# orhosko/tiny-ntt

Measured on AMD Instinct MI355X. Metric: negacyclic poly-mults/sec (n=4096, 60-bit q), bit-exact vs cg_ntt.py, higher is better.
Workload: dtype u64; 1 GPU; n=4096, q=2^60-2^14+1 (60-bit), global batch 65536 = 65536 rows on this GPU, LCG-seeded rows resident in HBM (BASELINE configs[2]); n=4096, q=1152921504606830593, rows_per_gpu=65536, global_batch=65536, variant=fused, kernel=polymul_fused_kernel, lazy_reduction=True, lib_build_id=33db21926526ecac, parallelism=batch-sharded x1, no data-path collective

## Files before the change

### tiny_ntt_amd/csrc/fused_core.h

```cpp
#pragma once
#include <type_traits>
#include "modarith.h"

#ifndef TN_ABL_UNIFORM_TW
#define TN_ABL_UNIFORM_TW 0
#endif

namespace tn {

template <int B, int E_, typename F> struct StaticFor {
  TN_HD static void run(F& f) { f(std::integral_constant<int, B>()); StaticFor<B + 1, E_, F>::run(f); }
};
template <int E_, typename F> struct StaticFor<E_, E_, F> { TN_HD static void run(F&) {} };
template <int B, int E_, typename F> TN_HD void static_for(F&& f) { StaticFor<B, E_, F>::run(f); }

#ifndef TN_FUSED_LPT10
#define TN_FUSED_LPT10 3
#endif
#ifndef TN_FUSED_LPT12
#define TN_FUSED_LPT12 3
#endif
constexpr int fused_lpt(int logn) {
  return logn == 8 ? 2 : logn == 9 ? 3 : logn == 10 ? TN_FUSED_LPT10 : logn == 11 ? 3 : logn == 12 ? TN_FUSED_LPT12 : logn == 13 ? 3 : 0;
}

template <typename E> struct Arith {
  E q;
  u64 mu;
  int k;
  u32 fold_c;
  SplitK sk;
  u64 qmul[17];
  typename TwOf<E>::type one;
  typename TwOf<E>::type ninv;
  typename TwOf<E>::type fninv;
  typename TwOf<E>::type fninv_w1;
  typename TwOf<E>::type bninv;
  typename TwOf<E>::type bninv_w1;
};

template <typename E, int LOGN_, int LPT_> struct FusedCfg {
  static constexpr int LOGN = LOGN_, LPT = LPT_;
  static constexpr int N = 1 << LOGN, R = 1 << LPT, THREADS = N >> LPT;
  static constexpr int PHASES = (LOGN + LPT - 1) / LPT;
  static constexpr int pos(int p) { return (LOGN - (p + 1) * LPT) < 0 ? 0 : (LOGN - (p + 1) * LPT); }
  static constexpr int stage_begin(int p) { return p * LPT; }
  static constexpr int stage_end(int p) { return ((p + 1) * LPT) < LOGN ? ((p + 1) * LPT) : LOGN; }
  static constexpr int ex_pad(int e) { return pos(e + 1) > 0 ? (1 << pos(e + 1)) : 1; }
  static constexpr int ex_sh(int e) { return pos(e + 1) > 0 ? pos(e + 1) + LPT : LPT; }
  static constexpr int lay_span(int e, int cnt) { return cnt + ex_pad(e) * (cnt >> ex_sh(e)); }
  static constexpr int WB = (LOGN - LPT > 6) ? (LOGN - LPT - 6) : 0;
  static constexpr int WSH = LOGN - WB;
  static constexpr int tau_bit_to_j(int p, int t) { return t < pos(p) ? t : t + LPT; }
  static constexpr bool ex_wave_local(int e) {
    for (int t = 6; t < LOGN - LPT; ++t)
      if (tau_bit_to_j(e, t) != t + LPT || tau_bit_to_j(e + 1, t) != t + LPT) return false;
    return true;
  }
  static constexpr int region_elems() {
    int m = 1 << WSH;
    for (int e = 0; e + 1 < PHASES; ++e)
      if (ex_wave_local(e) && lay_span(e, 1 << WSH) > m) m = lay_span(e, 1 << WSH);
    return m;
  }
  static constexpr int lds_elems() {
    int m = region_elems() << WB;
    for (int e = 0; e + 1 < PHASES; ++e)
      if (!ex_wave_local(e) && lay_span(e, N) > m) m = lay_span(e, N);
    return m;
  }
  TN_HD static constexpr u32 jidx(int p, u32 tau, u32 r) {
    return ((tau >> pos(p)) << (pos(p) + LPT)) | (r << pos(p)) | (tau & ((1u << pos(p)) - 1u));
  }
  TN_HD static constexpr u32 ex_addr(int e, u32 j) {
    if (WB > 0 && ex_wave_local(e))
      return (j >> WSH) * (u32)region_elems() + (j & ((1u << WSH) - 1u)) + (u32)ex_pad(e) * ((j & ((1u << WSH) - 1u)) >> ex_sh(e));
    return j + (u32)ex_pad(e) * (j >> ex_sh(e));
  }
  TN_HD static constexpr u32 ex_base(int e, int p, u32 tau) { return ex_addr(e, jidx(p, tau, 0)); }
  TN_HD static constexpr u32 ex_off(int e, int p, u32 r) { return ex_addr(e, jidx(p, 0, r)); }
  enum { TW_UNIFORM = 0, TW_WAVE = 1, TW_LDS = 2, TW_REGS = 3, TW_VEC = 4 };
  static constexpr int LDS_TW_MAX_STAGE = 9;
  static constexpr int tw_src(int p) {
    return pos(p) >= LOGN - LPT ? TW_UNIFORM
         : (pos(p) >= 6 ? TW_WAVE : (pos(p) > 0 ? (stage_end(p) <= LDS_TW_MAX_STAGE ? TW_LDS : TW_VEC) : TW_REGS));
  }
  static constexpr int lds_tw_lo() {
    for (int p = 0; p < PHASES; ++p) if (tw_src(p) == TW_LDS) return 1 << stage_begin(p);
    return 0;
  }
  static constexpr int lds_tw_hi() {
    int h = 0;
    for (int p = 0; p < PHASES; ++p) if (tw_src(p) == TW_LDS) h = 1 << stage_end(p);
    return h;
  }
  static constexpr int lds_tw_count() { return lds_tw_hi() - lds_tw_lo(); }
  static constexpr int pre_count(int s) { return R >> ((LOGN - 1 - s) - pos(PHASES - 1) + 1); }
  static constexpr int pre_off(int s) {
    int o = 0;
    for (int i = stage_begin(PHASES - 1); i < s; ++i) o += pre_count(i);
    return o;
  }
  static constexpr int NPRE = (tw_src(PHASES - 1) == TW_REGS) ? pre_off(LOGN) : 1;
  TN_HD static u32 nat_addr(u32 k) { return k ^ ((k >> 5) & 15u); }
  TN_HD static u32 thi(int p, u32 tau) {
    if (pos(p) >= LOGN - LPT) return 0u;
    if (pos(p) >= 6) return wave_uniform(tau >> pos(p));
    return tau >> pos(p);
  }
};

template <typename E> struct LazyTraits;
template <> struct LazyTraits<u64> { static constexpr int LIMIT = 16, TMUL = 4, PW = 2; };
template <> struct LazyTraits<u32> { static constexpr int LIMIT = 64, TMUL = 2, PW = 4; };

template <typename E, bool LAZY, bool CIN = false> struct Policy {
  typedef typename TwOf<E>::type Tw;
  static constexpr bool lazy = LAZY;
  static constexpr bool canonical_inputs = CIN && LAZY && sizeof(E) == 8;
  static constexpr bool split = LAZY && sizeof(E) == 8;
  static constexpr int LIMIT = LazyTraits<E>::LIMIT, TMUL = LazyTraits<E>::TMUL, PW = LazyTraits<E>::PW;

  TN_HD static E load(E x, const Arith<E>& ar) {
    if (canonical_inputs) return x;
    if (LAZY) return fold(x, ar.k, ar.fold_c);
    return mul_tw(x, ar.one, ar.q);
  }
  TN_HD static E canon(E x, const Arith<E>& ar) {
    if (LAZY) { x = fold(x, ar.k, ar.fold_c); return csub(x, ar.q); }
    return x;
  }
  template <int K> TN_HD static void ct(E& u, E& v, Tw w, const Arith<E>& ar) {
    if constexpr (split) {
      const u64 x = mul_sp_acc(u, v, w, ar.sk);
      v = ((u << 1) + ar.qmul[K]) - x;
      u = x;
    } else if constexpr (LAZY) {
      const E t = mul_tw_lazy(v, w, ar.q);
      v = u + ((E)K * ar.q - t);
      u = u + t;
    } else {
      E t = mul_tw(v, w, ar.q);
      E s = u + t;
      v = u >= t ? u - t : u + (ar.q - t);
      u = csub(s, ar.q);
    }
  }
  template <int BND> TN_HD static void gs(E& u, E& v, Tw w, const Arith<E>& ar) {
    if constexpr (split) {
      const E d = (u + ar.qmul[BND]) - v;
      u = u + v;
      v = mul_sp(d, w, ar.sk);
    } else if constexpr (LAZY) {
      const E d = u + ((E)BND * ar.q - v);
      u = u + v;
      v = mul_tw_lazy(d, w, ar.q);
    } else {
      E d = u >= v ? u - v : u + (ar.q - v);
      u = csub(u + v, ar.q);
      v = mul_tw(d, w, ar.q);
    }
  }
  template <int BND> TN_HD static void gs_last(E& u, E& v, const Arith<E>& ar) {
    E d;
    if constexpr (split) d = (u + ar.qmul[BND]) - v;
    else d = LAZY ? (E)(u + ((E)BND * ar.q - v)) : (u >= v ? (E)(u - v) : (E)(u + (ar.q - v)));
    E s = u + v;
    u = mul_tw_canon(s, ar.fninv, ar);
    v = mul_tw_canon(d, ar.fninv_w1, ar);
  }
  TN_HD static E mul_tw_canon(E a, Tw w, const Arith<E>& ar) {
    if constexpr (split) return csub(fold(mul_sp(a, w, ar.sk), ar.k, ar.fold_c), ar.q);
    else return mul_tw(a, w, ar.q);
  }
};

template <typename P, int LOGN> struct Sched {
  static constexpr int fwd_in(int s) {
    int b = 2;
    for (int i = 0; i < s; ++i) { if (b + P::TMUL > P::LIMIT) b = 2; b += P::TMUL; }
    return b;
  }
  static constexpr bool fwd_fold(int s) { return P::lazy && fwd_in(s) + P::TMUL > P::LIMIT; }
  static constexpr int fwd_out() {
    int b = 2;
    for (int i = 0; i < LOGN; ++i) { if (b + P::TMUL > P::LIMIT) b = 2; b += P::TMUL; }
    return b;
  }
  static constexpr int inv_in(int g) {
    int b = P::lazy ? P::PW : 1;
    for (int i = 0; i < g; ++i) { if (2 * b > P::LIMIT) b = 2; b = (2 * b > P::TMUL) ? 2 * b : P::TMUL; }
    return b;
  }
  static constexpr bool inv_fold(int g) { return P::lazy && 2 * inv_in(g) > P::LIMIT; }
  static constexpr int inv_bnd(int g) { return inv_fold(g) ? 2 : inv_in(g); }
};

template <typename Cfg, bool CIN = false, bool BC = false> struct SplitSched {
  static constexpr int LOGN = Cfg::LOGN, R = Cfg::R;
  static constexpr int FEND = BC ? LOGN - 1 : LOGN;
  static constexpr long U = 4096, CAP = 16 * U;
  static constexpr long FOLDED = U + 1;
  static constexpr long PW_OUT = 2 * U;
  static constexpr long PW_IN = 14 * (U - 1);
  static constexpr long tmax(long bv) { return 4 * U + (bv + 7) / 8 + 2; }
  static constexpr long BC_AMAX = CAP - 8;
  static constexpr int kq(long b) { return (int)((b + U - 2) / (U - 1)); }
  static constexpr int kf(long t) { return kq(t) <= 6 ? 6 : kq(t); }
  static constexpr int ki(long b) { return (kq(b) + 3) / 4 * 4; }
  static constexpr int phase_of(int s) { return s / Cfg::LPT; }
  static constexpr int bpos_of(int s) { return (LOGN - 1 - s) - Cfg::pos(phase_of(s)); }
  struct Data {
    bool ffold[LOGN][R] = {};
    unsigned char fk[LOGN][R] = {};
    long fout = 0;
    bool pw_fold_b = false;
    bool bcfold[R] = {};
    bool ifold[LOGN][R] = {};
    unsigned char ik[LOGN][R] = {};
  };
  static constexpr Data build() {
    Data d;
    long b[R] = {};
    for (int r = 0; r < R; ++r) b[r] = CIN ? U : (r < R / 2 ? FOLDED : CAP);
    for (int s = 0; s < FEND; ++s) {
      if (s > 0 && phase_of(s) != phase_of(s - 1)) {
        long m = 0;
        for (int r = 0; r < R; ++r) m = b[r] > m ? b[r] : m;
        for (int r = 0; r < R; ++r) b[r] = m;
      }
      const int bit = 1 << bpos_of(s);
      for (int r = 0; r < R; ++r) {
        if (r & bit) continue;
        const long t = tmax(b[r | bit]);
        const int K = kf(t);
        const long grow = t > K * U ? t : K * U;
        if (b[r] + grow > CAP) { d.ffold[s][r] = true; b[r] = FOLDED; }
        d.fk[s][r] = (unsigned char)K;
        const long bu = b[r];
        b[r] = bu + t;
        b[r | bit] = bu + K * U;
      }
    }
    for (int r = 0; r < R; ++r) d.fout = b[r] > d.fout ? b[r] : d.fout;
    d.pw_fold_b = d.fout > PW_IN;
    for (int r = 0; r < R; r += 2) {
      if (!BC) { b[r] = b[r + 1] = PW_OUT; continue; }
      long a0 = b[r], a1 = b[r + 1];
      if (a0 > BC_AMAX) { d.bcfold[r] = true; a0 = FOLDED; }
      if (a1 > BC_AMAX) { d.bcfold[r + 1] = true; a1 = FOLDED; }
      b[r] = tmax(a0) + tmax(tmax(a1));
      b[r + 1] = tmax(a0) + tmax(a1);
    }
    for (int g = BC ? 1 : 0; g < LOGN; ++g) {
      const int s = LOGN - 1 - g;
      if (g > 0 && phase_of(s) != phase_of(s + 1)) {
        long m = 0;
        for (int r = 0; r < R; ++r) m = b[r] > m ? b[r] : m;
        for (int r = 0; r < R; ++r) b[r] = m;
      }
      const int bit = 1 << bpos_of(s);
      for (int r = 0; r < R; ++r) {
        if (r & bit) continue;
        const int v = r | bit;
        for (int it = 0; it < 2; ++it) {
          if (b[r] + ki(b[v]) * U <= CAP && b[r] + b[v] <= CAP) break;
          if (b[r] >= b[v]) { d.ifold[g][r] = true; b[r] = FOLDED; }
          else { d.ifold[g][v] = true; b[v] = FOLDED; }
        }
        const int Kv = ki(b[v]);
        d.ik[g][r] = (unsigned char)Kv;
        const long bd = b[r] + Kv * U;
        b[r] = b[r] + b[v];
        b[v] = tmax(bd);
      }
    }
    return d;
  }
  static constexpr Data D = build();
};

template <typename Pol, typename Cfg, bool BC = false> struct SchedOf {
  typedef Sched<Pol, Cfg::LOGN> S;
  static constexpr bool fwd_fold(int s, int r) { return S::fwd_fold(s) && !(r & (1 << SplitSched<Cfg>::bpos_of(s))); }
  static constexpr int fwd_k(int, int) { return Pol::TMUL; }
  static constexpr bool inv_fold(int g, int) { return S::inv_fold(g); }
  static constexpr int inv_k(int g, int) { return S::inv_bnd(g); }
  static constexpr bool pw_fold_b() { return false; }
  static constexpr bool pw_ok() { return !Pol::lazy || S::fwd_out() <= Pol::LIMIT - 2; }
};
template <typename Cfg, bool CIN, bool BC> struct SchedOf<Policy<u64, true, CIN>, Cfg, BC> {
  typedef SplitSched<Cfg, CIN, BC> S;
  static constexpr bool fwd_fold(int s, int r) { return S::D.ffold[s][r]; }
  static constexpr int fwd_k(int s, int r) { return S::D.fk[s][r]; }
  static constexpr bool inv_fold(int g, int r) { return S::D.ifold[g][r]; }
  static constexpr int inv_k(int g, int r) { return S::D.ik[g][r]; }
  static constexpr bool pw_fold_b() { return S::D.pw_fold_b; }
  static constexpr bool pw_ok() { return true; }
  static constexpr bool bc_fold(int r) { return S::D.bcfold[r]; }
};

template <typename E> struct TwRefs {
  typedef typename TwOf<E>::type Tw;
  const Tw* __restrict__ glob;
  const Tw* lds;
  Tw* pre;
  const Tw* mid = nullptr;
  u32 zero = 0;
};

template <typename E, typename Cfg, int PH, int S_>
TN_HD typename TwOf<E>::type tw_get(const TwRefs<E>& t, u32 thi, int g) {
  constexpr int bpos = (Cfg::LOGN - 1 - S_) - Cfg::pos(PH);
  if (Cfg::tw_src(PH) == Cfg::TW_REGS) return t.pre[Cfg::pre_off(S_) + g];
  const u32 idx = (1u << S_) + (TN_ABL_UNIFORM_TW ? 0u : (thi << (Cfg::LPT - bpos - 1))) + (u32)g;
  if (Cfg::tw_src(PH) == Cfg::TW_LDS) {
    if (t.mid) return t.mid[(1 << (S_ - Cfg::stage_begin(PH))) - 1 + g];
    return t.lds[idx - Cfg::lds_tw_lo()];
  }
  if (Cfg::tw_src(PH) == Cfg::TW_VEC && t.mid) return t.mid[(1 << (S_ - Cfg::stage_begin(PH))) - 1 + g];
  return t.glob[idx + t.zero];
}

template <typename E, typename Cfg, int PH>
TN_HD void tw_fetch_vec(typename TwOf<E>::type (&mid)[Cfg::R], u32 tau, const typename TwOf<E>::type* __restrict__ glob) {
  const u32 thi = Cfg::thi(PH, tau);
  static_for<Cfg::stage_begin(PH), Cfg::stage_end(PH)>([&](auto s_) {
    constexpr int s = decltype(s_)::value;
    constexpr int bpos = (Cfg::LOGN - 1 - s) - Cfg::pos(PH);
    constexpr int cnt = Cfg::R >> (bpos + 1), off = (1 << (s - Cfg::stage_begin(PH))) - 1;
    const u32 boff = ((1u << s) + (thi << (Cfg::LPT - bpos - 1))) * (u32)sizeof(typename TwOf<E>::type);
    const typename TwOf<E>::type* base = reinterpret_cast<const typename TwOf<E>::type*>(reinterpret_cast<const char*>(glob) + boff);
#pragma unroll
    for (int g = 0; g < cnt; ++g) mid[off + g] = base[g];
  });
}

template <typename E, typename Cfg, int PH>
TN_HD void tw_fetch_mid(typename TwOf<E>::type (&mid)[Cfg::R], u32 tau, const typename TwOf<E>::type* lds_tw) {
  const u32 thi = Cfg::thi(PH, tau);
  static_for<Cfg::stage_begin(PH), Cfg::stage_end(PH)>([&](auto s_) {
    constexpr int s = decltype(s_)::value;
    constexpr int bpos = (Cfg::LOGN - 1 - s) - Cfg::pos(PH);
    constexpr int cnt = Cfg::R >> (bpos + 1), off = (1 << (s - Cfg::stage_begin(PH))) - 1;
#pragma unroll
    for (int g = 0; g < cnt; ++g)
      mid[off + g] = lds_tw[(1u << s) + (thi << (Cfg::LPT - bpos - 1)) + (u32)g - Cfg::lds_tw_lo()];
  });
}

template <typename E, typename Cfg, int S0, int S1>
TN_HD void tw_prefetch_stages(typename TwOf<E>::type* pre, u32 tau, const typename TwOf<E>::type* __restrict__ glob) {
  constexpr int PH = Cfg::PHASES - 1;
  if (Cfg::tw_src(PH) != Cfg::TW_REGS) return;
  const u32 thi = Cfg::thi(PH, tau);
  static_for<S0, S1>([&](auto s_) {
    constexpr int s = decltype(s_)::value;
    constexpr int bpos = (Cfg::LOGN - 1 - s) - Cfg::pos(PH);
    const u32 off = ((1u << s) + (thi << (Cfg::LPT - bpos - 1))) * (u32)sizeof(typename TwOf<E>::type);
    const typename TwOf<E>::type* base = reinterpret_cast<const typename TwOf<E>::type*>(reinterpret_cast<const char*>(glob) + off);
#pragma unroll
    for (int g = 0; g < Cfg::pre_count(s); ++g) pre[Cfg::pre_off(s) + g] = base[g];
  });
}
template <typename E, typename Cfg>
TN_HD void tw_prefetch_raw(typename TwOf<E>::type* pre, u32 tau, const typename TwOf<E>::type* __restrict__ glob) {
  tw_prefetch_stages<E, Cfg, Cfg::stage_begin(Cfg::PHASES - 1), Cfg::LOGN>(pre, tau, glob);
}

template <typename E, typename Cfg>
TN_HD void tw_prefetch(typename TwOf<E>::type (&pre)[Cfg::NPRE], u32 tau, const typename TwOf<E>::type* __restrict__ glob) {
  tw_prefetch_raw<E, Cfg>(pre, tau, glob);
}

template <typename E, typename Cfg, typename Pol, int PH, bool BC = false>
TN_HD void fwd_phase(E (&x)[Cfg::R], u32 tau, const TwRefs<E>& tw, const Arith<E>& ar) {
  typedef SchedOf<Pol, Cfg, BC> SO;
  typedef typename TwOf<E>::type Tw;
  const u32 thi = Cfg::thi(PH, tau);
  constexpr int SEND = BC && Cfg::stage_end(PH) == Cfg::LOGN ? Cfg::LOGN - 1 : Cfg::stage_end(PH);
  static_for<Cfg::stage_begin(PH), SEND>([&](auto s_) {
    constexpr int s = decltype(s_)::value;
    constexpr int bpos = (Cfg::LOGN - 1 - s) - Cfg::pos(PH);
    static_for<0, Cfg::R>([&](auto r_) {
      constexpr int r = decltype(r_)::value;
      if constexpr (Pol::lazy && SO::fwd_fold(s, r)) x[r] = fold(x[r], ar.k, ar.fold_c);
    });
    static_for<0, Cfg::R>([&](auto r_) {
      constexpr int r = decltype(r_)::value;
      if constexpr (!(r & (1 << bpos))) {
        const Tw w = tw_get<E, Cfg, PH, s>(tw, thi, r >> (bpos + 1));
        Pol::template ct<SO::fwd_k(s, r)>(x[r], x[r | (1 << bpos)], w, ar);
      }
    });
  });
}

template <typename E, typename Cfg, typename Pol, int PH, bool BC = false>
TN_HD void inv_phase(E (&x)[Cfg::R], u32 tau, const TwRefs<E>& tw, const Arith<E>& ar) {
  typedef SchedOf<Pol, Cfg, BC> SO;
  typedef typename TwOf<E>::type Tw;
  const u32 thi = Cfg::thi(PH, tau);
  constexpr int SEND = BC && Cfg::stage_end(PH) == Cfg::LOGN ? Cfg::LOGN - 1 : Cfg::stage_end(PH);
  static_for<0, SEND - Cfg::stage_begin(PH)>([&](auto i_) {
    constexpr int s = SEND - 1 - decltype(i_)::value;
    constexpr int g = Cfg::LOGN - 1 - s;
    constexpr int bpos = (Cfg::LOGN - 1 - s) - Cfg::pos(PH);
    static_for<0, Cfg::R>([&](auto r_) {
      constexpr int r = decltype(r_)::value;
      if constexpr (Pol::lazy && SO::inv_fold(g, r)) x[r] = fold(x[r], ar.k, ar.fold_c);
    });
    static_for<0, Cfg::R>([&](auto r_) {
      constexpr int r = decltype(r_)::value;
      if constexpr (!(r & (1 << bpos))) {
        constexpr int BND = SO::inv_k(g, r);
        if constexpr (s == 0) Pol::template gs_last<BND>(x[r], x[r | (1 << bpos)], ar);
        else {
          const Tw w = tw_get<E, Cfg, PH, s>(tw, thi, r >> (bpos + 1));
          Pol::template gs<BND>(x[r], x[r | (1 << bpos)], w, ar);
        }
      }
    });
  });
}

template <typename E, typename Cfg, typename Pol>
TN_HD void load_reduce(E (&x)[Cfg::R], const Arith<E>& ar) {
#pragma unroll
  for (int r = 0; r < Cfg::R / 2; ++r) x[r] = Pol::load(x[r], ar);
}

template <typename E, typename Cfg, int EX, int PH>
TN_HD void ex_store(const E (&x)[Cfg::R], u32 tau, E* lds) {
  E* base = lds + Cfg::ex_base(EX, PH, tau);
  static_for<0, Cfg::R>([&](auto r_) { constexpr int r = decltype(r_)::value; base[Cfg::ex_off(EX, PH, r)] = x[r]; });
}
template <typename E, typename Cfg, int EX, int PH>
TN_HD void ex_load(E (&x)[Cfg::R], u32 tau, const E* lds) {
  const E* base = lds + Cfg::ex_base(EX, PH, tau);
  static_for<0, Cfg::R>([&](auto r_) { constexpr int r = decltype(r_)::value; x[r] = base[Cfg::ex_off(EX, PH, r)]; });
}

TN_HD u64 pointwise_lazy(u64 a, u64 b, const Arith<u64>& ar) {
  return mulmod_solinas_lazy(fold(a, ar.k, ar.fold_c), b, ar.k, ar.fold_c);
}
TN_HD u32 pointwise_lazy(u32 a, u32 b, const Arith<u32>& ar) {
  return mulmod_barrett_lazy(fold(a, ar.k, ar.fold_c), fold(b, ar.k, ar.fold_c), ar.q, ar.mu, ar.k);
}
template <typename E, typename Cfg, typename Pol>
TN_HD void pointwise(E (&xa)[Cfg::R], const E (&xb)[Cfg::R], const Arith<E>& ar) {
  typedef SchedOf<Pol, Cfg> SO;
  static_assert(SO::pw_ok(), "pointwise_lazy: unfolded operand bound");
#pragma unroll
  for (int r = 0; r < Cfg::R; ++r) {
    if (Pol::lazy)
      xa[r] = pointwise_lazy(xa[r], SO::pw_fold_b() ? fold(xb[r], ar.k, ar.fold_c) : xb[r], ar);
    else
      xa[r] = mulmod_barrett(xa[r], xb[r], ar.q, ar.mu, ar.k);
    if (r & 1) sched_fence();
  }
}

TN_HD void basecase_pair(u64& a0, u64& a1, u64 b0, u64 b1, Tw64 zeta, const Arith<u64>& ar) {
  const Tw64 B0 = split_rec(b0, ar.k, ar.fold_c, ar.q), B1 = split_rec(b1, ar.k, ar.fold_c, ar.q);
  const u64 t = opaque64(mul_sp(a1, zeta, ar.sk));
  const u64 c0 = mul_sp_acc(opaque64(mul_sp(a0, B0, ar.sk)), t, B1, ar.sk);
  const u64 c1 = mul_sp_acc(opaque64(mul_sp(a0, B1, ar.sk)), a1, B0, ar.sk);
  a0 = c0;
  a1 = c1;
}
template <typename Cfg, typename Pol>
TN_HD void basecase(u64 (&xa)[Cfg::R], const u64 (&xb)[Cfg::R], const Tw64* zeta, const Arith<u64>& ar) {
  typedef SchedOf<Pol, Cfg, true> SO;
  static_assert(Pol::split && Cfg::pos(Cfg::PHASES - 1) == 0, "base case: split policy, pairs in neighbouring registers");
  static_for<0, Cfg::R / 2>([&](auto i_) {
    constexpr int r = 2 * decltype(i_)::value;
    if constexpr (SO::bc_fold(r)) xa[r] = fold(xa[r], ar.k, ar.fold_c);
    if constexpr (SO::bc_fold(r + 1)) xa[r + 1] = fold(xa[r + 1], ar.k, ar.fold_c);
    basecase_pair(xa[r], xa[r + 1], xb[r], xb[r + 1], zeta[r / 2], ar);
    sched_fence();
  });
}

}
```

### tiny_ntt_amd/csrc/modarith.h

```cpp
#pragma once
#include <stdint.h>

#if defined(__HIPCC__)
#define TN_HD __host__ __device__ __forceinline__
#else
#define TN_HD inline
#endif

namespace tn {

typedef uint32_t u32;
typedef uint64_t u64;

struct alignas(16) Tw64 { u64 w, wp; };
struct Tw32 { u32 w, wp; };

template <typename E> struct TwOf;
template <> struct TwOf<u64> { typedef Tw64 type; };
template <> struct TwOf<u32> { typedef Tw32 type; };

TN_HD u64 mulhi64(u64 a, u64 b) {
#if defined(__HIP_DEVICE_COMPILE__)
  return __umul64hi(a, b);
#else
  return (u64)(((unsigned __int128)a * b) >> 64);
#endif
}

TN_HD u64 opaque64(u64 x) {
#if defined(__HIP_DEVICE_COMPILE__)
  asm("" : "+v"(x));
#endif
  return x;
}
TN_HD u32 opaque32(u32 x) {
#if defined(__HIP_DEVICE_COMPILE__)
  asm("" : "+v"(x));
#endif
  return x;
}

TN_HD u32 opaque_copy(u32 x) {
#if defined(__HIP_DEVICE_COMPILE__)
  asm volatile("" : "+v"(x));
#endif
  return x;
}

TN_HD u32 opaque_zero() {
#if defined(__HIP_DEVICE_COMPILE__)
  u32 z;
  asm volatile("s_mov_b32 %0, 0" : "=s"(z));
  return z;
#else
  return 0;
#endif
}

TN_HD void sched_fence() {
#if defined(__HIP_DEVICE_COMPILE__)
  __builtin_amdgcn_sched_barrier(0);
#endif
}

TN_HD void sched_fence_valu() {
#if defined(__HIP_DEVICE_COMPILE__)
  __builtin_amdgcn_sched_barrier(0x0124);
#endif
}

TN_HD u32 wave_uniform(u32 x) {
#if defined(__HIP_DEVICE_COMPILE__)
  return (u32)__builtin_amdgcn_readfirstlane((int)x);
#else
  return x;
#endif
}

TN_HD u32 bitrev(u32 v, int bits) {
#if defined(__HIP_DEVICE_COMPILE__)
  return __brev(v) >> (32 - bits);
#else
  u32 r = 0;
  for (int i = 0; i < bits; ++i) { r = (r << 1) | (v & 1u); v >>= 1; }
  return r;
#endif
}

TN_HD u32 mulhi32(u32 a, u32 b) { return (u32)(((u64)a * b) >> 32); }

TN_HD u64 mulhi64_lo2(u64 a, u64 wp) {
  const u32 a0 = (u32)a, a1 = (u32)(a >> 32), p0 = (u32)wp, p1 = (u32)(wp >> 32);
  return ((u64)a1 * p1 + mulhi32(a0, p1)) + mulhi32(a1, p0);
}

TN_HD u64 mul_tw_acc(u64 u, u64 a, Tw64 t, u64 q) {
  const u64 qh = mulhi64_lo2(a, t.wp);
  const u64 nq = (u64)0 - q;
  const u32 a0 = (u32)a, a1 = (u32)(a >> 32), w0 = (u32)t.w, w1 = (u32)(t.w >> 32);
  const u32 h0 = (u32)qh, h1 = (u32)(qh >> 32), n0 = (u32)nq, n1 = (u32)(nq >> 32);
  u64 lo = (u64)a0 * w0 + u;
  lo = (u64)h0 * n0 + lo;
  u64 hi = (u64)a0 * w1;
  hi = (u64)a1 * w0 + hi;
  hi = (u64)h0 * n1 + hi;
  hi = (u64)h1 * n0 + hi;
  hi = opaque64(hi);
  const u32 rh = opaque32((u32)(lo >> 32) + (u32)hi);
  return ((u64)rh << 32) | (u32)lo;
}

TN_HD u64 mul_tw_lazy(u64 a, Tw64 t, u64 q) { return mul_tw_acc(0, a, t, q); }

TN_HD u64 csub(u64 x, u64 q) { return x >= q ? x - q : x; }

TN_HD u64 mul_tw(u64 a, Tw64 t, u64 q) {
  u64 r = mul_tw_lazy(a, t, q);
  r = csub(r, 2 * q);
  return csub(r, q);
}

struct SplitK { u32 mulp, cf; };
#ifndef TN_SOLINAS5
#define TN_SOLINAS5 0
#endif
#if TN_SOLINAS5
TN_HD u64 mul_sp_acc(u64 u, u64 a, Tw64 t, SplitK sk) {
  const u32 a0 = (u32)a, a1 = (u32)(a >> 32);
  const u32 w0 = (u32)t.w, w1 = (u32)(t.w >> 32), x0 = (u32)t.wp, x1 = (u32)(t.wp >> 32);
  const u64 L1 = (u64)a0 * w0;
  const u64 H1 = (u64)a0 * w1 + (L1 >> 32);
  const u64 L2 = (u64)a1 * x0 + (u32)L1;
  const u64 H2 = (u64)a1 * x1 + (H1 + (L2 >> 32));
  const u32 top = (u32)(H2 >> 30);
  const u64 low = ((u64)((u32)H2 & 0x3FFFFFFFu) << 32) | (u32)L2;
  return u + (low + (u64)top * (sk.cf << 1));
}
#else
TN_HD u64 mul_sp_acc(u64 u, u64 a, Tw64 t, SplitK sk) {
  const u32 a0 = (u32)a, a1 = (u32)(a >> 32);
  u64 L = (u64)a0 * (u32)t.w + u;
  L = (u64)a1 * (u32)t.wp + L;
  u64 H = (u64)a0 * (u32)(t.w >> 32);
  H = (u64)a1 * (u32)(t.wp >> 32) + H;
  u64 r = (u64)(u32)H * sk.mulp + L;
  r = (u64)(u32)(H >> 32) * sk.cf + r;
  return r;
}
#endif
TN_HD u64 mul_sp(u64 a, Tw64 t, SplitK sk) { return mul_sp_acc(0, a, t, sk); }

TN_HD u64 mulmod_barrett(u64 a, u64 b, u64 q, u64 mu, int k) {
  u64 plo = a * b, phi = mulhi64(a, b);
  u64 q1 = (k - 1 == 0) ? plo : ((phi << (64 - (k - 1))) | (plo >> (k - 1)));
  u64 mlo = q1 * mu, mhi = mulhi64(q1, mu);
  u64 q2 = (mhi << (64 - (k + 1))) | (mlo >> (k + 1));
  u64 r = plo - q2 * q;
  r = csub(r, q);
  return csub(r, q);
}

TN_HD u64 fold(u64 x, int k, u32 c) {
  const u32 top = (u32)(x >> 32) >> (k - 32);
  const u64 lowmask = ((u64)((1u << (k - 32)) - 1u) << 32) | 0xFFFFFFFFull;
  return (x & lowmask) + (u64)top * c;
}

TN_HD Tw64 split_rec(u64 b, int k, u32 c, u64 q) {
  const u64 w = csub(fold(b, k, c), q);
  const int s = k - 32, p = k - 31;
  const u32 mp = (1u << p) - 1u;
  const u64 xl = (u64)(u32)(w >> s) * c;
  const u32 xh = opaque32((u32)(xl >> 32) + ((u32)w & ((1u << s) - 1u)));
  const u64 x = ((u64)xh << 32) | (u32)xl;
  Tw64 t;
  t.w = ((u64)(u32)(w >> p) << 32) | ((u32)w & mp);
  t.wp = ((u64)(u32)(x >> p) << 32) | ((u32)x & mp);
  return t;
}

TN_HD u64 mulmod_solinas_lazy(u64 a, u64 b, int k, u32 c) {
  const int s = k - 32;
  const u32 ms = (1u << s) - 1u;
  const u32 a0 = (u32)a, a1 = (u32)(a >> 32), b0 = (u32)b, b1 = (u32)(b >> 32);
  const u64 m0 = (u64)a0 * b0;
  const u64 m1 = (u64)a0 * b1 + (m0 >> 32);
  const u64 m2 = (u64)a1 * b0 + (u32)m1;
  const u64 m3 = (u64)a1 * b1 + (m1 >> 32) + (m2 >> 32);
  const u32 p0 = (u32)m0, p1 = (u32)m2;
  const u32 ph0 = (u32)((((u64)(u32)m3 << 32) | p1) >> s);
  const u32 ph1 = (u32)(m3 >> s);
  const u64 pl = ((u64)(p1 & ms) << 32) | p0;
  const u64 t = (u64)ph0 * c + pl;
  const u64 u = (u64)ph1 * c;
  const u32 uh = (u32)(u >> s);
  const u32 vh = (u32)(t >> 32) + ((u32)u & ms);
  const u32 top = (vh >> s) + uh;
  return (((u64)(vh & ms) << 32) | (u32)t) + (u64)top * c;
}

TN_HD u32 mul_tw_lazy(u32 a, Tw32 t, u32 q) {
  u32 qh = (u32)(((u64)a * t.wp) >> 32);
  return a * t.w - qh * q;
}

TN_HD u32 csub(u32 x, u32 q) { return x >= q ? x - q : x; }

TN_HD u32 mul_tw(u32 a, Tw32 t, u32 q) { return csub(mul_tw_lazy(a, t, q), q); }

TN_HD u32 mulmod_barrett(u32 a, u32 b, u32 q, u64 mu, int k) {
  u64 p = (u64)a * b;
  u64 q1 = p >> (k - 1);
  u64 q2 = (q1 * mu) >> (k + 1);
  u32 r = (u32)p - (u32)q2 * q;
  r = csub(r, q);
  return csub(r, q);
}

TN_HD u32 mulmod_barrett_lazy(u32 a, u32 b, u32 q, u64 mu, int k) {
  u64 p = (u64)a * b;
  u64 q1 = p >> (k - 1);
  u64 q2 = (q1 * mu) >> (k + 1);
  return (u32)p - (u32)q2 * q;
}

TN_HD u32 fold(u32 x, int k, u32 c) {
  u32 lowmask = (((u32)1) << k) - 1;
  return (x & lowmask) + (x >> k) * c;
}

inline u64 h_mulmod(u64 a, u64 b, u64 q) { return (u64)(((unsigned __int128)a * b) % q); }
inline u64 h_powmod(u64 b, u64 e, u64 q) {
  u64 r = 1 % q; b %= q;
  while (e) { if (e & 1) r = h_mulmod(r, b, q); b = h_mulmod(b, b, q); e >>= 1; }
  return r;
}
inline int h_bitlen(u64 x) { int n = 0; while (x) { ++n; x >>= 1; } return n; }
inline Tw64 h_make_tw64(u64 w, u64 q) {
  Tw64 t; t.w = w; t.wp = (u64)((((unsigned __int128)w) << 64) / q); return t;
}
inline Tw64 h_make_tw64_split(u64 w, u64 q, int k) {
#if TN_SOLINAS5
  Tw64 t5; t5.w = w; t5.wp = (u64)((((unsigned __int128)w) << 32) % q); (void)k; return t5;
#endif
  const int p = k - 31;
  const u64 x = (u64)((((unsigned __int128)w) << 32) % q), m = (((u64)1) << p) - 1;
  Tw64 t; t.w = (w & m) | ((w >> p) << 32); t.wp = (x & m) | ((x >> p) << 32); return t;
}
inline u64 h_split_value(Tw64 t, int k) { return TN_SOLINAS5 ? t.w : (u64)(u32)t.w + ((t.w >> 32) << (k - 31)); }
inline Tw32 h_make_tw32(u64 w, u64 q) {
  Tw32 t; t.w = (u32)w; t.wp = (u32)((w << 32) / q); return t;
}
inline bool h_is_prime(u64 n) {
  if (n < 2) return false;
  static const u64 small[] = {2, 3, 5, 7, 11, 13, 17, 19, 23, 29, 31, 37};
  for (u64 p : small) { if (n == p) return true; if (n % p == 0) return false; }
  u64 d = n - 1; int s = 0;
  while ((d & 1) == 0) { d >>= 1; ++s; }
  for (u64 a : small) {
    u64 x = h_powmod(a, d, n);
    if (x == 1 || x == n - 1) continue;
    bool comp = true;
    for (int i = 1; i < s; ++i) { x = h_mulmod(x, x, n); if (x == n - 1) { comp = false; break; } }
    if (comp) return false;
  }
  return true;
}

}
```

### tiny_ntt_amd/csrc/plan_tables.h

```cpp
#pragma once
#include <vector>
#include "launch_plan.h"

namespace tn {

struct HostTables {
  u32 n = 0, logn = 0;
  u64 q = 0, psi = 0, omega = 0, mu = 0;
  int k = 0, elem_bytes = 8;
  bool lazy = false;
  bool cg_lazy = false;
  bool cg_sched = false;
  bool cin_ok = false;
  bool bc_ok = false;
  u32 fold_c = 0;
  u64 n_inv = 0, ninv_w1 = 0;
  u64 n2_inv = 0, n2inv_w1 = 0;
  std::vector<u64> psi_pow, psi_inv_pow, psi_inv_ninv, psi_brv, psi_inv_brv, omega_pow, omega_inv_pow;
  std::vector<u64> cyc_brv, cyc_inv_brv;
  std::vector<u64> psi_bc, cyc_bc;
};

inline u32 h_brv(u32 v, u32 bits) {
  u32 r = 0;
  for (u32 i = 0; i < bits; ++i) { r = (r << 1) | (v & 1); v >>= 1; }
  return r;
}

inline bool h_lazy_ok(u64 q, int elem_bytes, u32* fold_c) {
  const int W = elem_bytes * 8, k = h_bitlen(q);
  const unsigned __int128 two_w = ((unsigned __int128)1) << W;
  const int LIMIT = elem_bytes == 8 ? LazyTraits<u64>::LIMIT : LazyTraits<u32>::LIMIT;
  const u64 c = (((u64)1) << k) - q;
  const bool fits = (unsigned __int128)LIMIT * q <= two_w;
  const unsigned __int128 top = (two_w >> k);
  const bool fold_ok = c < ((u64)1 << 32) && (unsigned __int128)c * (top + 1) <= q && (elem_bytes == 4 || k >= 32);
  if (fold_c) *fold_c = (fits && fold_ok) ? (u32)c : 0;
  return fits && fold_ok;
}

inline bool h_pw_fast_ok(u64 q, int k, u64 c) {
  typedef unsigned __int128 u128;
  if (k < 32 || k > 60 || c == 0 || c >= ((u64)1 << 31)) return false;
  const int s = k - 32;
  const u128 one = 1, w64 = one << 64, w32 = one << 32;
  const u128 amax = (one << k) - 1 + ((one << (64 - k)) - 1) * c;
  if (amax >= (one << 62)) return false;
  const u128 bmax = (u128)(LazyTraits<u64>::LIMIT - 2) * q;
  if (bmax >= w64) return false;
  const u128 pmax = amax * bmax;
  const u128 phmax = pmax >> k;
  if (phmax >= w64) return false;
  const u128 ph1max = phmax >> 32;
  const u128 umax = ph1max * c;
  if (umax >= w64) return false;
  const u128 uhmax = umax >> s;
  const u128 tmax = (one << k) - 1 + (w32 - 1) * c;
  if (tmax >= w64) return false;
  const u128 vhmax = (tmax >> 32) + ((one << s) - 1);
  if (vhmax >= w32) return false;
  const u128 topmax = (vhmax >> s) + uhmax;
  if (topmax >= w32) return false;
  const u128 rmax = (one << k) - 1 + topmax * c;
  return rmax < (u128)2 * q;
}

struct SplitExact {
  typedef unsigned __int128 u128;
  int k, p;
  u64 q, c, cf;
  u128 two64;
  bool ok = true;
  SplitExact(int k_, u64 c_) : k(k_), p(k_ - 31), c(c_) {
    q = (((u64)1) << k) - c;
    two64 = ((u128)1) << 64;
    cf = p >= 1 ? (u64)((((u128)1) << (p + 32)) % q) : 0;
    if (k < 32 || k > 60 || cf >= ((u64)1 << 32) || c >= ((u64)1 << 32)) ok = false;
  }
  u128 tmax(u128 bv) { return tmax_rec(bv, (u128)((q - 1) >> p), (u128)((q - 1) >> p)); }
  u128 tmax_rec(u128 bv, u128 whi, u128 xhi) {
    const u128 m32 = (((u128)1) << 32) - 1;
    u128 a1 = (bv - 1) >> 32; if (a1 > m32) a1 = m32;
    const u128 lo = (((u128)1) << p) - 1;
    const u128 H = m32 * whi + a1 * xhi;
    if (H >= two64 || whi > m32 || xhi > m32) ok = false;
    return m32 * lo + a1 * lo + (m32 << p) + (H >> 32) * cf + 1;
  }
  u128 rec_whi() { return (u128)((q - 1) >> p); }
  u128 rec_xhi() {
    const u128 xmax = (((((u128)1) << 32) - 1) * c) + (((((u128)1) << (k - 32)) - 1) << 32);
    if (xmax >= two64) ok = false;
    return xmax >> p;
  }
  u128 folded(u128 b) { return (((u128)1) << k) + ((b - 1) >> k) * c; }
  void fits(u128 exclusive) { if (exclusive > two64) ok = false; }
};

template <typename Cfg, bool CIN = false, bool BC = false> inline bool h_split_sched_replay(int k, u64 c) {
  typedef SplitSched<Cfg, CIN, BC> S;
  typedef unsigned __int128 u128;
  SplitExact x(k, c);
  if (!x.ok) return false;
  constexpr int R = Cfg::R, LOGN = Cfg::LOGN;
  const auto& D = S::D;
  u128 b[R];
  auto level = [&]() { u128 m = 0; for (int r = 0; r < R; ++r) m = b[r] > m ? b[r] : m; for (int r = 0; r < R; ++r) b[r] = m; };
  for (int r = 0; r < R; ++r) b[r] = CIN ? (u128)x.q : (r < R / 2 ? x.folded(x.two64) : x.two64);
  for (int s = 0; s < S::FEND; ++s) {
    if (s > 0 && S::phase_of(s) != S::phase_of(s - 1)) level();
    const int bit = 1 << S::bpos_of(s);
    for (int r = 0; r < R; ++r) {
      if (r & bit) continue;
      if (D.ffold[s][r]) b[r] = x.folded(b[r]);
      const u128 t = x.tmax(b[r | bit]), kq = (u128)D.fk[s][r] * x.q;
      if (kq + 1 < t) x.ok = false;
      x.fits(b[r] - 1 + t); x.fits(b[r] + kq);
      const u128 bu = b[r];
      b[r] = bu + t - 1; b[r | bit] = bu + kq;
    }
  }
  u128 fout = 0, fo[R];
  for (int r = 0; r < R; ++r) { fout = b[r] > fout ? b[r] : fout; fo[r] = b[r]; }
  if (x.folded(fout) > (u128)2 * x.q) x.ok = false;
  if (!D.pw_fold_b && fout > (u128)14 * x.q) x.ok = false;
  for (int r = 0; r < R; ++r) b[r] = (u128)2 * x.q;
  if (x.folded(x.two64) > (u128)2 * x.q) x.ok = false;
  if (BC) {
    const u128 whi = x.rec_whi(), xhi = x.rec_xhi();
    for (int r = 0; r < R; r += 2) {
      const u128 a0 = D.bcfold[r] ? x.folded(fo[r]) : fo[r], a1 = D.bcfold[r + 1] ? x.folded(fo[r + 1]) : fo[r + 1];
      const u128 t = x.tmax(a1);
      const u128 p0 = x.tmax_rec(a0, whi, xhi), p1 = x.tmax_rec(t, whi, xhi), p2 = x.tmax_rec(a1, whi, xhi);
      x.fits(p0 + p1 - 1); x.fits(p0 + p2 - 1);
      b[r] = p0 + p1 - 1;
      b[r + 1] = p0 + p2 - 1;
    }
  }
  for (int g = BC ? 1 : 0; g < LOGN; ++g) {
    const int s = LOGN - 1 - g;
    if (g > 0 && S::phase_of(s) != S::phase_of(s + 1)) level();
    const int bit = 1 << S::bpos_of(s);
    for (int r = 0; r < R; ++r) if (D.ifold[g][r]) b[r] = x.folded(b[r]);
    for (int r = 0; r < R; ++r) {
      if (r & bit) continue;
      const int v = r | bit;
      const u128 kq = (u128)D.ik[g][r] * x.q;
      if (kq + 1 < b[v]) x.ok = false;
      x.fits(b[r] + kq); x.fits(b[r] + b[v] - 1);
      const u128 bd = b[r] + kq;
      b[r] = b[r] + b[v] - 1;
      b[v] = x.tmax(bd);
    }
  }
  if (x.folded(x.tmax(x.two64)) > (u128)2 * x.q) x.ok = false;
  return x.ok;
}

inline bool h_cg_lazy_ok(int k, u64 c) {
  typedef unsigned __int128 u128;
  SplitExact x(k, c);
  if (!x.ok) return false;
  const u128 bu = x.folded(x.two64);
  const u128 kq = (u128)6 * x.q;
  const u128 B = bu + kq;
  const u128 t = x.tmax(B);
  if (kq + 1 < t) x.ok = false;
  x.fits(bu - 1 + t); x.fits(B);
  if (bu + t - 1 > B) x.ok = false;
  if (x.folded(B) > (u128)2 * x.q) x.ok = false;
  if (x.tmax(x.two64) > B) x.ok = false;
  if (B > (u128)14 * (x.q - 1)) x.ok = false;
  {
    const u128 t1 = x.tmax(x.two64), k7 = (u128)7 * x.q;
    if (k7 + 1 < t1) x.ok = false;
    x.fits(bu - 1 + t1); x.fits(bu + k7);
    const u128 out1 = (bu + t1 - 1) > (bu + k7) ? (bu + t1 - 1) : (bu + k7);
    const u128 t2 = x.tmax(out1);
    if (kq + 1 < t2) x.ok = false;
    x.fits(bu - 1 + t2);
    if (bu + t2 - 1 > B) x.ok = false;
  }
  return x.ok;
}

inline bool h_cg_sched_ok(int k, u64 c) {
  typedef unsigned __int128 u128;
  SplitExact x(k, c);
  if (!x.ok) return false;
  u128 b_odd = x.tmax(x.two64);
  const u128 fold_any = x.folded(x.two64);
  if (fold_any > b_odd) b_odd = fold_any;
  u128 out_merged = 0;
  {
    const u128 bl = x.tmax(x.two64), t1 = x.tmax(x.two64), k7 = (u128)7 * x.q;
    if (k7 + 1 < t1) x.ok = false;
    x.fits(bl - 1 + t1); x.fits(bl + k7);
    out_merged = (bl + t1 - 1) > (bl + k7) ? (bl + t1 - 1) : (bl + k7);
  }
  for (int it = 0; it < 4; ++it) {
    const u128 t1 = x.tmax(b_odd), k5 = (u128)5 * x.q;
    if (k5 + 1 < t1) x.ok = false;
    x.fits(b_odd - 1 + t1); x.fits(b_odd + k5);
    const u128 s1 = b_odd + t1 - 1, d1 = b_odd + k5;
    u128 b_even = s1 > d1 ? s1 : d1;
    if (out_merged > b_even) b_even = out_merged;
    const u128 bu = x.folded(b_even), t2 = x.tmax(b_even), k6 = (u128)6 * x.q;
    if (k6 + 1 < t2) x.ok = false;
    x.fits(bu - 1 + t2); x.fits(bu + k6);
    const u128 s2 = bu + t2 - 1, d2 = bu + k6;
    const u128 out = s2 > d2 ? s2 : d2;
    if (out <= b_odd) {
      if (b_odd > (u128)14 * (x.q - 1)) x.ok = false;
      if (x.folded(b_odd) > (u128)2 * x.q) x.ok = false;
      return x.ok;
    }
    b_odd = out;
  }
  return false;
}

inline bool h_split_sched_cin_ok(u32 logn, int k, u64 c) {
  return logn == 12 && h_split_sched_replay<FusedCfg<u64, 12, fused_lpt(12)>, true>(k, c);
}

inline bool h_bc_sched_ok(u32 logn, int k, u64 c) {
  constexpr int L = FUSED_BC_LOGN;
  return (int)logn == L && fused_has_bc<u64, L, fused_lpt(L), true>() && h_split_sched_replay<FusedCfg<u64, L, fused_lpt(L)>, false, true>(k, c);
}

inline bool h_split_sched_ok(u32 logn, int k, u64 c) {
  switch (logn) {
    case 8: return h_split_sched_replay<FusedCfg<u64, 8, fused_lpt(8)>>(k, c);
    case 9: return h_split_sched_replay<FusedCfg<u64, 9, fused_lpt(9)>>(k, c);
    case 10: return h_split_sched_replay<FusedCfg<u64, 10, fused_lpt(10)>>(k, c);
    case 11: return h_split_sched_replay<FusedCfg<u64, 11, fused_lpt(11)>>(k, c);
    case 12: return h_split_sched_replay<FusedCfg<u64, 12, fused_lpt(12)>>(k, c);
    case 13: return h_split_sched_replay<FusedCfg<u64, 13, fused_lpt(13)>>(k, c);
    default: return false;
  }
}

inline HostTables h_build_tables(u32 n, u64 q, u64 psi, bool allow_lazy) {
  HostTables t;
  u32 logn = 0;
  while (((u32)1 << logn) < n) ++logn;
  t.n = n; t.logn = logn; t.q = q; t.psi = psi % q; t.omega = h_mulmod(t.psi, t.psi, q);
  t.elem_bytes = q < ((u64)1 << 31) ? 4 : 8;
  t.k = h_bitlen(q);
  t.mu = (u64)((((unsigned __int128)1) << (2 * t.k)) / q);
  t.lazy = h_lazy_ok(q, t.elem_bytes, &t.fold_c) && allow_lazy;
  if (t.lazy && t.elem_bytes == 8 && !h_pw_fast_ok(q, t.k, t.fold_c)) t.lazy = false;
  if (t.lazy && t.elem_bytes == 8 && !h_split_sched_ok(logn, t.k, t.fold_c)) t.lazy = false;
  if (!t.lazy) t.fold_c = 0;
  t.cg_lazy = t.lazy && t.elem_bytes == 8 && h_cg_lazy_ok(t.k, t.fold_c);
  t.cg_sched = t.cg_lazy && (logn & 1) == 0 && h_cg_sched_ok(t.k, t.fold_c);
  t.cin_ok = t.lazy && t.elem_bytes == 8 && h_split_sched_cin_ok(logn, t.k, t.fold_c);
  t.bc_ok = t.lazy && t.elem_bytes == 8 && h_bc_sched_ok(logn, t.k, t.fold_c);
  const u64 psi_inv = h_powmod(t.psi, q - 2, q);
  const u64 omega_inv = h_powmod(t.omega, q - 2, q);
  t.n_inv = h_powmod(n % q, q - 2, q);
  std::vector<u64>& psi_inv_pow = t.psi_inv_pow;
  psi_inv_pow.resize(n);
  t.psi_pow.resize(n); t.psi_inv_ninv.resize(n); t.psi_brv.resize(n); t.psi_inv_brv.resize(n);
  t.omega_pow.resize(n / 2 + 1); t.omega_inv_pow.resize(n / 2 + 1);
  u64 f = 1, g = 1;
  for (u32 i = 0; i < n; ++i) { t.psi_pow[i] = f; psi_inv_pow[i] = g; f = h_mulmod(f, t.psi, q); g = h_mulmod(g, psi_inv, q); }
  for (u32 i = 0; i < n; ++i) {
    t.psi_brv[i] = t.psi_pow[h_brv(i, logn)];
    t.psi_inv_brv[i] = psi_inv_pow[h_brv(i, logn)];
    t.psi_inv_ninv[i] = h_mulmod(psi_inv_pow[i], t.n_inv, q);
  }
  t.cyc_brv.assign(n, 1); t.cyc_inv_brv.assign(n, 1);
  for (u32 i = 1; i < n; ++i) {
    u32 m = 1;
    while (2 * m <= i) m *= 2;
    const u32 e = h_brv(i, logn) - n / (2 * m);
    t.cyc_brv[i] = t.psi_pow[e];
    t.cyc_inv_brv[i] = psi_inv_pow[e];
  }
  u64 w = 1, wi = 1;
  for (u32 j = 0; j <= n / 2; ++j) { t.omega_pow[j] = w; t.omega_inv_pow[j] = wi; w = h_mulmod(w, t.omega, q); wi = h_mulmod(wi, omega_inv, q); }
  t.ninv_w1 = h_mulmod(t.n_inv, t.psi_inv_brv[1], q);
  t.n2_inv = h_mulmod(t.n_inv, 2, q);
  t.n2inv_w1 = h_mulmod(t.n2_inv, t.psi_inv_brv[1], q);
  if (t.bc_ok) {
    t.psi_bc = t.psi_brv; t.cyc_bc = t.cyc_brv;
    for (u32 i = n / 2; i < n; ++i) { t.psi_bc[i] = h_mulmod(t.psi_brv[i], t.psi_brv[i], q); t.cyc_bc[i] = h_mulmod(t.cyc_brv[i], t.cyc_brv[i], q); }
  }
  return t;
}

inline HostTables h_build_omega_tables(u32 n, u64 q, u64 omega) {
  HostTables t;
  u32 logn = 0;
  while (((u32)1 << logn) < n) ++logn;
  t.n = n; t.logn = logn; t.q = q; t.psi = 0; t.omega = omega % q;
  t.elem_bytes = q < ((u64)1 << 31) ? 4 : 8;
  t.k = h_bitlen(q);
  t.mu = (u64)((((unsigned __int128)1) << (2 * t.k)) / q);
  t.lazy = false; t.cg_lazy = false; t.fold_c = 0;
  const u64 omega_inv = h_powmod(t.omega, q - 2, q);
  t.n_inv = h_powmod(n % q, q - 2, q);
  t.omega_pow.resize(n / 2 + 1); t.omega_inv_pow.resize(n / 2 + 1);
  u64 w = 1 % q, wi = 1 % q;
  for (u32 j = 0; j <= n / 2; ++j) { t.omega_pow[j] = w; t.omega_inv_pow[j] = wi; w = h_mulmod(w, t.omega, q); wi = h_mulmod(wi, omega_inv, q); }
  t.ninv_w1 = t.n_inv;
  return t;
}

inline HostTables h_build_general_tables(u32 n, u64 q, u64 psi) {
  HostTables t;
  u32 logn = 0;
  while (((u32)1 << logn) < n) ++logn;
  t.n = n; t.logn = logn; t.q = q; t.psi = psi % q; t.omega = h_mulmod(t.psi, t.psi, q);
  t.elem_bytes = q < ((u64)1 << 31) ? 4 : 8;
  t.k = h_bitlen(q);
  t.mu = (u64)((((unsigned __int128)1) << (2 * t.k)) / q);
  t.lazy = false; t.cg_lazy = false; t.cg_sched = false; t.fold_c = 0;
  const u64 psi_inv = h_powmod(t.psi, q - 2, q), omega_inv = h_powmod(t.omega, q - 2, q);
  t.n_inv = h_powmod(n % q, q - 2, q);
  t.psi_pow.resize(n); t.psi_inv_pow.resize(n); t.psi_inv_ninv.resize(n);
  u64 f = 1 % q, g = 1 % q;
  for (u32 i = 0; i < n; ++i) {
    t.psi_pow[i] = f; t.psi_inv_pow[i] = g; t.psi_inv_ninv[i] = h_mulmod(g, t.n_inv, q);
    f = h_mulmod(f, t.psi, q); g = h_mulmod(g, psi_inv, q);
  }
  t.omega_pow.resize(n / 2 + 1); t.omega_inv_pow.resize(n / 2 + 1);
  u64 w = 1 % q, wi = 1 % q;
  for (u32 j = 0; j <= n / 2; ++j) { t.omega_pow[j] = w; t.omega_inv_pow[j] = wi; w = h_mulmod(w, t.omega, q); wi = h_mulmod(wi, omega_inv, q); }
  t.ninv_w1 = t.n_inv;
  return t;
}

template <typename E> inline typename TwOf<E>::type h_make_tw(u64 w, u64 q);
template <> inline Tw64 h_make_tw<u64>(u64 w, u64 q) { return h_make_tw64(w, q); }
template <> inline Tw32 h_make_tw<u32>(u64 w, u64 q) { return h_make_tw32(w, q); }

template <typename E> inline std::vector<typename TwOf<E>::type> h_tw_table(const std::vector<u64>& v, u64 q) {
  std::vector<typename TwOf<E>::type> t(v.size());
  for (size_t i = 0; i < v.size(); ++i) t[i] = h_make_tw<E>(v[i], q);
  return t;
}

inline bool h_uses_split(const HostTables& t) { return t.lazy && t.elem_bytes == 8; }
template <typename E> inline typename TwOf<E>::type h_make_fused_tw(u64 w, const HostTables& t) { return h_make_tw<E>(w, t.q); }
template <> inline Tw64 h_make_fused_tw<u64>(u64 w, const HostTables& t) {
  return h_uses_split(t) ? h_make_tw64_split(w, t.q, t.k) : h_make_tw64(w, t.q);
}
template <typename E> inline std::vector<typename TwOf<E>::type> h_fused_table(const std::vector<u64>& v, const HostTables& t) {
  std::vector<typename TwOf<E>::type> r(v.size());
  for (size_t i = 0; i < v.size(); ++i) r[i] = h_make_fused_tw<E>(v[i], t);
  return r;
}

template <typename E> inline Arith<E> h_make_arith(const HostTables& t) {
  Arith<E> ar;
  ar.q = (E)t.q; ar.mu = t.mu; ar.k = t.k; ar.fold_c = t.fold_c;
  ar.sk.mulp = 0; ar.sk.cf = 0;
  for (int K = 0; K <= 16; ++K) ar.qmul[K] = (u64)(((unsigned __int128)K * t.q) & ~(u64)0);
  if (h_uses_split(t)) {
    const int p = t.k - 31;
    ar.sk.mulp = (u32)1 << p;
    ar.sk.cf = (u32)((((unsigned __int128)1) << (p + 32)) % t.q);
  }
  ar.one = h_make_tw<E>(1, t.q);
  ar.ninv = h_make_tw<E>(t.n_inv, t.q);
  ar.fninv = h_make_fused_tw<E>(t.n_inv, t);
  ar.fninv_w1 = h_make_fused_tw<E>(t.ninv_w1, t);
  ar.bninv = h_make_fused_tw<E>(t.n2_inv, t);
  ar.bninv_w1 = h_make_fused_tw<E>(t.n2inv_w1, t);
  return ar;
}

}
```

Baseline: 30.01 million poly-mults/s.

## Use lazy split reciprocals and power-of-two conditional subtract in base case

Replaces the fully reduced split_rec in the base-case pair multiply with a lazy variant that only double-folds the operand, skipping the final canonical reduction. Adds a csub_pow2 that does the conditional subtraction of q=2^k-c with 32-bit ops via a carry bit instead of a 64-bit compare-subtract, used in canon and mul_tw_canon. Tightens the lazy-bound fold multipliers when the base case is on, and updates the host bound replay to check the wider reciprocal input range. This removes some 64-bit integer work per element, but correctness now depends on the new bound analysis.

```diff
diff --git a/tiny_ntt_amd/csrc/fused_core.h b/tiny_ntt_amd/csrc/fused_core.h
--- a/tiny_ntt_amd/csrc/fused_core.h
+++ b/tiny_ntt_amd/csrc/fused_core.h
@@ -127,8 +127,9 @@
     return mul_tw(x, ar.one, ar.q);
   }
   TN_HD static E canon(E x, const Arith<E>& ar) {
-    if (LAZY) { x = fold(x, ar.k, ar.fold_c); return csub(x, ar.q); }
-    return x;
+    if constexpr (split) return csub_pow2(fold(x, ar.k, ar.fold_c), ar.k, ar.fold_c);
+    else if constexpr (LAZY) { x = fold(x, ar.k, ar.fold_c); return csub(x, ar.q); }
+    else return x;
   }
   template <int K> TN_HD static void ct(E& u, E& v, Tw w, const Arith<E>& ar) {
     if constexpr (split) {
@@ -170,7 +171,7 @@
     v = mul_tw_canon(d, ar.fninv_w1, ar);
   }
   TN_HD static E mul_tw_canon(E a, Tw w, const Arith<E>& ar) {
-    if constexpr (split) return csub(fold(mul_sp(a, w, ar.sk), ar.k, ar.fold_c), ar.q);
+    if constexpr (split) return csub_pow2(fold(mul_sp(a, w, ar.sk), ar.k, ar.fold_c), ar.k, ar.fold_c);
     else return mul_tw(a, w, ar.q);
   }
 };
@@ -206,8 +207,8 @@
   static constexpr long tmax(long bv) { return 4 * U + (bv + 7) / 8 + 2; }
   static constexpr long BC_AMAX = CAP - 8;
   static constexpr int kq(long b) { return (int)((b + U - 2) / (U - 1)); }
-  static constexpr int kf(long t) { return kq(t) <= 6 ? 6 : kq(t); }
-  static constexpr int ki(long b) { return (kq(b) + 3) / 4 * 4; }
+  static constexpr int kf(long t) { return BC ? kq(t) : (kq(t) <= 6 ? 6 : kq(t)); }
+  static constexpr int ki(long b) { return BC ? kq(b) : (kq(b) + 3) / 4 * 4; }
   static constexpr int phase_of(int s) { return s / Cfg::LPT; }
   static constexpr int bpos_of(int s) { return (LOGN - 1 - s) - Cfg::pos(phase_of(s)); }
   struct Data {
@@ -462,7 +463,7 @@
 }
 
 TN_HD void basecase_pair(u64& a0, u64& a1, u64 b0, u64 b1, Tw64 zeta, const Arith<u64>& ar) {
-  const Tw64 B0 = split_rec(b0, ar.k, ar.fold_c, ar.q), B1 = split_rec(b1, ar.k, ar.fold_c, ar.q);
+  const Tw64 B0 = split_rec_lazy(b0, ar.k, ar.fold_c), B1 = split_rec_lazy(b1, ar.k, ar.fold_c);
   const u64 t = opaque64(mul_sp(a1, zeta, ar.sk));
   const u64 c0 = mul_sp_acc(opaque64(mul_sp(a0, B0, ar.sk)), t, B1, ar.sk);
   const u64 c1 = mul_sp_acc(opaque64(mul_sp(a0, B1, ar.sk)), a1, B0, ar.sk);
diff --git a/tiny_ntt_amd/csrc/modarith.h b/tiny_ntt_amd/csrc/modarith.h
--- a/tiny_ntt_amd/csrc/modarith.h
+++ b/tiny_ntt_amd/csrc/modarith.h
@@ -177,6 +177,28 @@
   t.w = ((u64)(u32)(w >> p) << 32) | ((u32)w & mp);
   t.wp = ((u64)(u32)(x >> p) << 32) | ((u32)x & mp);
   return t;
+}
+
+TN_HD Tw64 split_rec_lazy(u64 b, int k, u32 c) {
+  const u64 w = fold(fold(b, k, c), k, c);
+  const int s = k - 32, p = k - 31;
+  const u32 mp = (1u << p) - 1u;
+  const u64 xl = (u64)(u32)(w >> s) * c;
+  const u32 xh = opaque32((u32)(xl >> 32) + ((u32)w & ((1u << s) - 1u)));
+  const u64 x = ((u64)xh << 32) | (u32)xl;
+  Tw64 t;
+  t.w = ((u64)(u32)(w >> p) << 32) | ((u32)w & mp);
+  t.wp = ((u64)(u32)(x >> p) << 32) | ((u32)x & mp);
+  return t;
+}
+
+TN_HD u64 csub_pow2(u64 y, int k, u32 c) {
+  const u64 z = y + c;
+  const u32 zh = (u32)(z >> 32), bit = 1u << (k - 32);
+  const bool ge = (zh & bit) != 0;
+  const u32 hi = ge ? (zh & (bit - 1u)) : (u32)(y >> 32);
+  const u32 lo = ge ? (u32)z : (u32)y;
+  return ((u64)hi << 32) | lo;
 }
 
 TN_HD u64 mulmod_solinas_lazy(u64 a, u64 b, int k, u32 c) {
diff --git a/tiny_ntt_amd/csrc/plan_tables.h b/tiny_ntt_amd/csrc/plan_tables.h
--- a/tiny_ntt_amd/csrc/plan_tables.h
+++ b/tiny_ntt_amd/csrc/plan_tables.h
@@ -86,7 +86,11 @@
     if (H >= two64 || whi > m32 || xhi > m32) ok = false;
     return m32 * lo + a1 * lo + (m32 << p) + (H >> 32) * cf + 1;
   }
-  u128 rec_whi() { return (u128)((q - 1) >> p); }
+  u128 rec_whi() {
+    const u128 twok = ((u128)1) << k, over = folded(two64) - twok;
+    if (over + c >= twok) ok = false;
+    return (twok - 1) >> p;
+  }
   u128 rec_xhi() {
     const u128 xmax = (((((u128)1) << 32) - 1) * c) + (((((u128)1) << (k - 32)) - 1) << 32);
     if (xmax >= two64) ok = false;
```

Measured after the change: 29.76 million poly-mults/s. No clear change (-0.8%).
